# myrrix/myrrix-recommender

Hardware: AMD Instinct MI355X
Metric: ALS rows solved/sec (full iteration) at k=64 (higher is better)
Workload: dtype f32 storage; per-row Gramian: f16x2-split operands (22 bits), f32 accumulate; Cholesky f32

## Files before the change

myrrix-recommender_amd/csrc/als_kernels.h:

```cpp
#pragma once
#include <hip/hip_runtime.h>
#include <stdint.h>

#include <type_traits>

#include "work_plan.h"

namespace mals {

#ifndef MALS_WAVES
#define MALS_WAVES(T, MODE) ((T) <= 4 ? 4 : ((T) == 5 ? 3 : 2))
#endif
#ifndef MALS_WAVES_H
#define MALS_WAVES_H(T, MODE) ((T) <= 2 ? 5 : ((T) <= 4 ? 3 : 2))
#endif

typedef float f32x4 __attribute__((ext_vector_type(4)));
typedef double f64x4 __attribute__((ext_vector_type(4)));

__host__ __device__ constexpr int tri(int T) { return T * (T + 1) / 2; }
__host__ __device__ constexpr int tidx(int T, int i, int j) { return i * T - (i * (i - 1)) / 2 + (j - i); }

constexpr int GRAMIAN_FLUSH_BINADES = 5;
constexpr int YMAX_SLOTS = 64;
// ... 853 lines not shown
    } else {
#pragma unroll
      for (int r = 0; r < 4; ++r) acc[t][r] *= s2;
    }
  }
#pragma unroll
  for (int v = 0; v < T; ++v) bcol[v] *= s2;
  return inv_s2;
}

template <int T, bool PERM = false>
__device__ __forceinline__ void store_row(const SolveParams& p, float (&xcol)[T], float minpiv, float wmax, int row, int lane) {
  if (!(minpiv > p.sing_threshold)) {
    if (lane == 0) {
      if (p.refine_flag) {
        p.refine_flag[row] = 2;
        *p.any_marked = 1;
      } else {
        atomicMin(p.bad_row, (unsigned long long)row);
      }
    }
#pragma unroll
    for (int v = 0; v < T; ++v) xcol[v] = 0.f;
  } else {
    if (minpiv <= 1024.f * p.sing_threshold && lane == 0) {
      const unsigned long long key = ((unsigned long long)__float_as_uint(minpiv) << 32) | (unsigned)row;
      if (key < __builtin_nontemporal_load(p.suspect)) atomicMin(p.suspect, key);
    }
    if (p.refine_flag && p.refine_limit > 0.f && wmax > p.refine_limit * minpiv && lane == 0) {
      p.refine_flag[row] = 1;
      *p.any_marked = 1;
    }
  }
  if constexpr (PERM) {
    static_assert(T == 8, "the permuted feature order belongs to the k = 128 kernels");
    float* o = p.out + (int64_t)row * p.k;
    int l2 = lane;
    asm volatile("" : "+v"(l2));
    const int g = l2 >> 4, c = l2 & 15;
    const bool hi = ((g ^ (c >> 3)) & 1) != 0;
    f32x4 x;
#pragma unroll
    for (int q = 0; q < 4; ++q) x[q] = hi ? xcol[4 + q] : xcol[q];
    if (g < 2) *reinterpret_cast<f32x4*>(o + 8 * c + 4 * g) = x;
  } else {
    float* o = p.out + (int64_t)row * p.k;
    int l2 = lane;
    asm volatile("" : "+v"(l2));
    const int g = l2 >> 4, c = l2 & 15;
#pragma unroll
    for (int m = 0; 4 * m < T; ++m) {
      const float x = select4(g, xcol[4 * m], 4 * m + 1 < T ? xcol[4 * m + 1] : 0.f, 4 * m + 2 < T ? xcol[4 * m + 2] : 0.f,
                              4 * m + 3 < T ? xcol[4 * m + 3] : 0.f);
      const int feat = 16 * (4 * m + g) + c;
      if (4 * m + 3 < T - 1 || feat < p.k) o[feat] = x;
    }
  }
}

template <int T, bool PERM = false>
__device__ __forceinline__ void finish_row(const SolveParams& p, f32x4 (&acc)[tri(T)], const float (&bcol)[T],
                                           int n_u, int row, int lane, float rmax = 0.f) {
  add_ridge<T, PERM>(p, acc, n_u, lane);
  float minpiv = 3.0e38f;
  float xcol[T];
  const float wmax = fmaxf(rmax, p.gramian_weight * __int_as_float(max_entry_bits<T>(acc, lane)));
  cholesky_tiles<T>(acc, lane, minpiv);
  solve_tiles<T>(acc, bcol, xcol, lane);
// ... 1098 lines not shown
```

myrrix-recommender_amd/csrc/lds_kernels.h:

```cpp
#pragma once
#include "als_kernels.h"

namespace mals {

constexpr int LDSK_T = 8, LDSK_E = 8;
#ifndef MALS_LDSK_RESPLIT
#define MALS_LDSK_RESPLIT 1
#endif
constexpr bool LDSK_RESPLIT = MALS_LDSK_RESPLIT != 0;
constexpr int LDSK_ROW_BYTES = 512;
constexpr int LDSK_RING_BYTES = 32 * LDSK_ROW_BYTES;
constexpr int LDSK_CHUNK_BYTES = 512;
constexpr int LDSK_NCHUNK = 3;
constexpr int LDSK_WAVE_BYTES = LDSK_RING_BYTES + LDSK_NCHUNK * LDSK_CHUNK_BYTES;

__host__ __device__ constexpr int ldsk_feature(int v, int c) { return 8 * c + (v ^ (4 * (c >> 3))); }

typedef __attribute__((address_space(3))) char lds_char;

__device__ __forceinline__ void glds16(const void* a, unsigned dst) {
  unsigned keep;
  asm volatile(
      "s_mov_b32 %0, m0\n\t"
      "s_mov_b32 m0, %2\n\ts_nop 0\n\tglobal_load_lds_dwordx4 %1, off\n\t"
      "s_mov_b32 m0, %0"
      : "=&s"(keep)
      : "v"(a), "s"(dst)
      : "memory");
}
__device__ __forceinline__ void glds4x2(const void* a0, const void* a1, unsigned dst) {
  unsigned keep;
  const unsigned d1 = dst + 256;
  asm volatile(
      "s_mov_b32 %0, m0\n\t"
      "s_mov_b32 m0, %3\n\ts_nop 0\n\tglobal_load_lds_dword %1, off nt\n\t"
      "s_mov_b32 m0, %4\n\ts_nop 0\n\tglobal_load_lds_dword %2, off nt\n\t"
      "s_mov_b32 m0, %0"
      : "=&s"(keep)
      : "v"(a0), "v"(a1), "s"(dst), "s"(d1)
      : "memory");
}
template <int N>
__device__ __forceinline__ void wait_vm() {
  asm volatile("s_waitcnt vmcnt(%0)" ::"n"(N) : "memory");
}

typedef const __attribute__((address_space(3))) f32x4* lds_f4;
typedef const __attribute__((address_space(3))) i32x4* lds_i4;
typedef const __attribute__((address_space(3))) float* lds_f1;

struct LdskLane {
  unsigned rd0;
  const char* gsrc;
};

__device__ __forceinline__ void ldsk_chunk_dma(const SolveParams& p, int64_t begin, int len, int base, unsigned buf, int lane) {
  const int n = base + lane;
  const int nn = n < len ? n : len - 1;
  glds4x2(p.col + begin + nn, p.val + begin + nn, buf);
}

__device__ __forceinline__ void ldsk_weights(const SolveParams& p, const lds_char* lds, unsigned buf, int base, int len, int lane, float zscale,
                                             float& w, float& cb) {
  const int widx = 4 * (lane & 15) + (lane >> 4);
  Chunk e;
  e.col = 0;
  e.w = *reinterpret_cast<lds_f1>(lds + buf + 256 + 4 * widx);
  e.cb = base + widx < len ? 1.f : 0.f;
  chunk_weights_h(p, e, zscale);
  w = e.w;
  cb = e.cb;
}

template <int E2>
__device__ __forceinline__ void ldsk_issue_pair(const lds_char* lds, unsigned ring, unsigned cols_at, const LdskLane& L) {
  const i32x4 cols = *reinterpret_cast<lds_i4>(lds + cols_at + 32 * E2);
#pragma unroll
  for (int i = 0; i < 4; ++i) {
    const char* a;
    asm("v_mad_u64_u32 %0, vcc, %1, %2, %3" : "=v"(a) : "v"(cols[i]), "s"((unsigned)LDSK_ROW_BYTES), "v"(L.gsrc) : "vcc");
    glds16(a, ring + 4096 * E2 + 1024 * i);
  }
}
__device__ __forceinline__ unsigned ldsk_cols_addr(unsigned buf_cols, int lane) { return buf_cols + 16 * (unsigned)(lane >> 5); }

template <int E2, int V0>
__device__ __forceinline__ void ldsk_convert_half(const f32x4& ya, const f32x4& yb, float s0, float s1, float c0, float c1,
                                                  ZOp<LDSK_E> (&zh)[LDSK_T], ZOp<LDSK_E> (&zl)[LDSK_T], float (&bpart)[LDSK_T]) {
#pragma unroll
  for (int q = 0; q < 4; ++q) {
    const int v = V0 + q;
    const float y0 = ya[q], y1 = yb[q];
    const float z0 = y0 * s0, z1 = y1 * s1;
    const int hp = pk_rn16(z0, z1);
    const f16x2 hh = __builtin_bit_cast(f16x2, hp);
    zh[v].r[E2] = hp;
    zl[v].r[E2] = pk_rn16(fmaf((float)hh[0], -1.f, z0), fmaf((float)hh[1], -1.f, z1));
    bpart[v] = fmaf(c0, y0, bpart[v]);
    bpart[v] = fmaf(c1, y1, bpart[v]);
  }
}

template <int E2>
__device__ __forceinline__ void ldsk_pair(const lds_char* lds, unsigned ring, float w, float cb, unsigned next_cols, const LdskLane& L,
                                          ZOp<LDSK_E> (&zh)[LDSK_T], ZOp<LDSK_E> (&zl)[LDSK_T], float (&bpart)[LDSK_T]) {
  wait_vm<12>();
  const float s0 = row_bcast<2 * E2>(w), s1 = row_bcast<2 * E2 + 1>(w);
  const float c0 = row_bcast<2 * E2>(cb), c1 = row_bcast<2 * E2 + 1>(cb);
  {
    const f32x4 ya = *reinterpret_cast<lds_f4>(lds + L.rd0 + 4096 * E2);
    const f32x4 yb = *reinterpret_cast<lds_f4>(lds + L.rd0 + 4096 * E2 + 512);
    ldsk_convert_half<E2, 0>(ya, yb, s0, s1, c0, c1, zh, zl, bpart);
  }
  __builtin_amdgcn_sched_barrier(0);
  {
    const f32x4 ya = *reinterpret_cast<lds_f4>(lds + (L.rd0 ^ 16u) + 4096 * E2);
    const f32x4 yb = *reinterpret_cast<lds_f4>(lds + (L.rd0 ^ 16u) + 4096 * E2 + 512);
    ldsk_convert_half<E2, 4>(ya, yb, s0, s1, c0, c1, zh, zl, bpart);
  }
  __builtin_amdgcn_sched_barrier(0);
  ldsk_issue_pair<E2>(lds, ring, next_cols, L);
  __builtin_amdgcn_sched_barrier(0);
}
__device__ __forceinline__ void ldsk_super_step(const lds_char* lds, unsigned ring, float w, float cb, unsigned next_cols, const LdskLane& L,
                                                f32x4 (&acc)[tri(LDSK_T)], float (&bpart)[LDSK_T]) {
  ZOp<LDSK_E> zh[LDSK_T], zl[LDSK_T];
  ldsk_pair<0>(lds, ring, w, cb, next_cols, L, zh, zl, bpart);
  ldsk_pair<1>(lds, ring, w, cb, next_cols, L, zh, zl, bpart);
  ldsk_pair<2>(lds, ring, w, cb, next_cols, L, zh, zl, bpart);
  ldsk_pair<3>(lds, ring, w, cb, next_cols, L, zh, zl, bpart);
  gram_super_step<LDSK_T, LDSK_E>(zh, zl, acc);
  __builtin_amdgcn_sched_barrier(0);
}

__global__ void gramian_perm_kernel(const double* __restrict__ G, int k, float* __restrict__ Gp) {
  constexpr int T = LDSK_T;
  const int e = blockIdx.x * blockDim.x + threadIdx.x;
  if (e >= tri(T) * 256) return;
  const int t = e >> 8, lane = (e >> 2) & 63, reg = e & 3;
  int i = 0, rem = t;
  while (rem >= T - i) {
    rem -= T - i;
    ++i;
  }
  const int j = i + rem;
  const int row = ldsk_feature(i, 4 * (lane >> 4) + reg), col = ldsk_feature(j, lane & 15);
  Gp[e] = (row < k && col < k) ? (float)G[(int64_t)row * k + col] : 0.f;
}

template <int MODE>
__global__ __launch_bounds__(64, 2) void als_lds_kernel_h(SolveParams p) {
  constexpr int T = LDSK_T;
  __shared__ __attribute__((aligned(1024))) char lds_raw[LDSK_WAVE_BYTES];
  const lds_char* lds = (const lds_char*)lds_raw;
  const unsigned lbase = (unsigned)(uintptr_t)lds;
  const int lane = threadIdx.x;
  const int64_t wave = blockIdx.x, n_waves = gridDim.x;
  int64_t it = wave;
  if (it >= p.n_work) return;
  if (p.zscale[2] == 0.f) return;
  const float zscale = __int_as_float(uniform(__float_as_int(p.zscale[0])));
  const float inv_s2 = __int_as_float(uniform(__float_as_int(p.zscale[1])));
  LdskLane L;
  {
    const int g = lane >> 4, c = lane & 15;
    L.rd0 = (unsigned)(g * 1024 + 32 * c + 16 * (c >> 3));
    L.gsrc = reinterpret_cast<const char*>(p.M) + 16 * (lane & 31);
  }
  const unsigned ring = lbase;
  unsigned b_cur = LDSK_RING_BYTES, b_next = LDSK_RING_BYTES + LDSK_CHUNK_BYTES, b_nrow = LDSK_RING_BYTES + 2 * LDSK_CHUNK_BYTES;
  const f32x4* Gp4 = reinterpret_cast<const f32x4*>(p.Gperm);
  WorkItem cur = load_item(p, it);
  WorkItem nxt = load_item(p, it + n_waves);
  WorkItem nx2 = load_item(p, it + 2 * n_waves);
  if (cur.len > 0) {
    ldsk_chunk_dma(p, cur.begin, cur.len, 0, lbase + b_cur, lane);
    if (nxt.len > 0) ldsk_chunk_dma(p, nxt.begin, nxt.len, 0, lbase + b_nrow, lane);
    wait_vm<0>();
    {
      const unsigned ca = ldsk_cols_addr(b_cur, lane);
      ldsk_issue_pair<0>(lds, ring, ca, L);
      ldsk_issue_pair<1>(lds, ring, ca, L);
      ldsk_issue_pair<2>(lds, ring, ca, L);
      ldsk_issue_pair<3>(lds, ring, ca, L);
    }
    for (;;) {
      const WorkItem nx3 = load_item(p, it + 3 * n_waves);
      f32x4 acc[tri(T)];
#pragma unroll
      for (int t = 0; t < tri(T); ++t) acc[t] = f32x4{0.f, 0.f, 0.f, 0.f};
      float bpart[T];
#pragma unroll
      for (int v = 0; v < T; ++v) bpart[v] = 0.f;
#ifdef MALS_PROFILING
      const int64_t trow = it / n_waves - p.trace_start;
      const bool tr = MODE == 0 && p.trace && wave < 64 && trow >= 0 && trow < 64;
      unsigned long long t0 = 0, t1 = 0, t2 = 0;
      if (tr) t0 = __builtin_readcyclecounter();
#endif
      wait_vm<0>();
      const int n_ss = (cur.len + 31) >> 5;
      float w = 0.f, cb = 0.f;
      for (int ss = 0; ss < n_ss; ++ss) {
        const bool odd = ss & 1, last = ss + 1 == n_ss;
        if (!odd) {
          if (ss > 0) {
            const unsigned t = b_cur;
            b_cur = b_next;
            b_next = t;
          }
          ldsk_weights(p, lds, b_cur, 32 * ss, cur.len, lane, zscale, w, cb);
          if (32 * ss + 64 < cur.len) ldsk_chunk_dma(p, cur.begin, cur.len, 32 * ss + 64, lbase + b_next, lane);
        } else {
          w = row_ror<8>(w);
          cb = row_ror<8>(cb);
        }
        const unsigned src = last ? (nxt.len > 0 ? b_nrow : b_cur) : (odd ? b_next : b_cur + 128);
        ldsk_super_step(lds, ring, w, cb, ldsk_cols_addr(src, lane), L, acc, bpart);
      }
#ifdef MALS_PROFILING
      if (tr) t1 = __builtin_readcyclecounter();
#endif
      float bcol[T];
#pragma unroll
      for (int v = 0; v < T; ++v) bcol[v] = reduce_groups(bpart[v], lane);
      {
        const unsigned t = b_cur;
        b_cur = b_nrow;
        b_nrow = t;
      }
      if (nx2.len > 0) ldsk_chunk_dma(p, nx2.begin, nx2.len, 0, lbase + b_nrow, lane);
      if (MODE == 0) {
        const float rmax = p.refine_flag ? __int_as_float(max_entry_bits<T>(acc, lane)) * inv_s2 : 0.f;
        {
          int l2 = lane;
          asm volatile("" : "+v"(l2));
#pragma unroll
          for (int t0 = 0; t0 < tri(T); t0 += 9) {
            f32x4 g4[9];
#pragma unroll
            for (int t = 0; t < 9; ++t) g4[t] = Gp4[(t0 + t) * 64 + l2];
#pragma unroll
            for (int t = 0; t < 9; ++t)
#pragma unroll
              for (int r = 0; r < 4; ++r) acc[t0 + t][r] = fmaf(acc[t0 + t][r], inv_s2, g4[t][r]);
            __builtin_amdgcn_sched_barrier(0);
          }
        }
        add_ridge<T, true>(p, acc, cur.len, lane);
        float minpiv = 3.0e38f, wmax;
        float xcol[T];
        const float inv_s2row = row_scale<T>(acc, bcol, lane, wmax);
        cholesky_tiles<T, true, LDSK_RESPLIT, true>(acc, lane, minpiv);
        minpiv *= inv_s2row;
#ifdef MALS_PROFILING
        if (tr) t2 = __builtin_readcyclecounter();
#endif
        solve_tiles<T>(acc, bcol, xcol, lane);
        store_row<T, true>(p, xcol, minpiv, fmaxf(rmax, p.gramian_weight * wmax), cur.id, lane);
#ifdef MALS_PROFILING
        if (tr) {
          const unsigned long long t3 = __builtin_readcyclecounter();
          if (lane == 0) {
            unsigned long long* o = p.trace + (trow * 64 + wave) * 6;
            o[0] = t0; o[1] = t1; o[2] = t2; o[3] = t3; o[4] = (unsigned long long)cur.len; o[5] = wall_clock64();
          }
        }
#endif
      } else {
        float* s = p.scratch + (int64_t)cur.id * ((tri(T) * 4 + T) * 64);
#pragma unroll
        for (int t = 0; t < tri(T); ++t) reinterpret_cast<f32x4*>(s)[t * 64 + lane] = acc[t] * inv_s2;
#pragma unroll
        for (int v = 0; v < T; ++v) s[(tri(T) * 4 + v) * 64 + lane] = bcol[v];
      }
      cur = nxt;
      nxt = nx2;
      nx2 = nx3;
      it += n_waves;
      if (cur.len <= 0) break;
    }
    wait_vm<0>();
  }
  if (MODE == 0) {
    while (cur.len == 0) {
      f32x4 acc[tri(T)];
#pragma unroll
      for (int t = 0; t < tri(T); ++t) acc[t] = Gp4[t * 64 + lane];
      float bcol[T];
#pragma unroll
      for (int v = 0; v < T; ++v) bcol[v] = 0.f;
      finish_row<T, true>(p, acc, bcol, 0, cur.id, lane);
      it += n_waves;
      cur = load_item(p, it);
    }
  }
}

}
```

myrrix-recommender_amd/csrc/mals_api.hip:

```cpp
#include "../../include/myrrix_als.h"
#include "als_kernels.h"
#include "dual_kernels.h"
#include "lds_kernels.h"
#include "host_eigen.h"
#include "host_solver.h"
#include "mals_internal.h"
#include "mals_handle.h"
#include "hip_buffer.h"
#include "work_plan.h"
#include "convergence.h"

#include <hip/hip_runtime.h>

#include <algorithm>
#include <chrono>
#include <cmath>
#include <cstdio>
#include <cstdlib>
#include <cstring>
#include <limits>
#include <new>
#include <string>
#include <type_traits>
#include <vector>
// ... 270 lines not shown
    double* pd = reinterpret_cast<double*>(s.partials.get() + 2 * slab_bytes);
    int* has2 = reinterpret_cast<int*>(s.partials.get() + 2 * slab_bytes + sizeof(double) * (size_t)GROUPS * tri(T) * 256);
    hipLaunchKernelGGL((gramian_split_kernel<T, false>), dim3((unsigned)(n_slabs / 4)), dim3(256), 0, h->stream, M, n_rows, k,
                       slab_rows, pf, has2, ymax);
    hipLaunchKernelGGL((gramian_split_kernel<T, true>), dim3((unsigned)(n_slabs / 4)), dim3(256), 0, h->stream, M, n_rows, k,
                       slab_rows, pf2, has2, ymax);
    hipLaunchKernelGGL(gramian_reduce_slabs_kernel, dim3((unsigned)((elems + 255) / 256), GROUPS), dim3(256), 0, h->stream, pf, pf2, has2, n_slabs,
                       elems, GROUPS, pd);
    hipLaunchKernelGGL((gramian_finalize_kernel<T, false>), dim3(elems / 64), dim3(256), 0, h->stream, pd, (int64_t)GROUPS, k, G_out, Gf_out);
    HIPCHK(h, hipGetLastError());
    return MALS_OK;
  }
  int64_t n_waves = std::min<int64_t>(1024, std::max<int64_t>(1, (n_rows + 63) / 64));
  n_waves = (n_waves + 3) & ~(int64_t)3;
  int64_t rows_per_wave = (n_rows + n_waves - 1) / n_waves;
  rows_per_wave = std::max<int64_t>(4, (rows_per_wave + 3) & ~(int64_t)3);
  const size_t bytes = sizeof(double) * (size_t)n_waves * tri(T) * 256;
  if (s.partials.capacity() < bytes) HIPCHK(h, s.partials.alloc(bytes));
  double* partials = reinterpret_cast<double*>(s.partials.get());
  if (ymax) HIPCHK(h, hipMemsetAsync(ymax, 0x7f, sizeof(unsigned), h->stream));
  hipLaunchKernelGGL((gramian_partial_kernel<T>), dim3((unsigned)(n_waves / 4)), dim3(256), 0, h->stream, M, n_rows, k,
                     rows_per_wave, partials);
  hipLaunchKernelGGL((gramian_finalize_kernel<T, true, 16>), dim3(elems / 16), dim3(256), 0, h->stream, partials, n_waves,
                     k, G_out, Gf_out);
  HIPCHK(h, hipGetLastError());
  return MALS_OK;
}

int launch_gramian(mals_handle h, SideState& s, const float* M, int64_t n_rows, double* G_out, float* Gf_out, unsigned* ymax = nullptr) {
  return dispatch_T(h, [&](auto t) { return launch_gramian_T<t()>(h, s, M, n_rows, G_out, Gf_out, ymax); });
}

template <typename K>
int persistent_grid(mals_handle h, K kernel, int64_t n_work, unsigned* grid, bool front = false, int block = 256, int resident_per_cu = 0) {
  const int64_t groups = (n_work + block / 64 - 1) / (block / 64);
  if (front) {
    *grid = (unsigned)std::max<int64_t>(1, groups);
    return MALS_OK;
  }
  int per_cu = resident_per_cu;
  if (!per_cu) HIPCHK(h, hipOccupancyMaxActiveBlocksPerMultiprocessor(&per_cu, kernel, 256, 0));
  if (per_cu < 1) per_cu = 1;
  per_cu *= 16;
  if (const char* e = std::getenv("MALS_BLOCKS_PER_CU")) per_cu = std::max(1, std::atoi(e)) * (256 / block);
  const int64_t cap = (int64_t)h->n_cu * per_cu;
  *grid = (unsigned)std::max<int64_t>(1, std::min<int64_t>(groups, cap));
  return MALS_OK;
}

enum { LISTS_ROWS = 1, LISTS_DUAL_ROWS = 2, LISTS_LONG = 4 };

template <typename KR, typename KS, typename KRF, typename KSF, typename KC, typename KCF, typename KP>
struct ListKernels {
  KR rows;
  KS segments;
  KRF rows_f32;
  KSF segments_f32;
  KC finish;
  KCF finish_f32;
  KP prereduce;
  int block;
  int resident_per_cu;
};
template <typename KR, typename KS, typename KRF, typename KSF, typename KC, typename KCF, typename KP>
ListKernels(KR, KS, KRF, KSF, KC, KCF, KP, int, int) -> ListKernels<KR, KS, KRF, KSF, KC, KCF, KP>;

template <typename K, typename KF>
int launch_persistent(mals_handle h, K kernel, KF fallback, int block, int resident_per_cu, const SolveParams& p, int kind, double bytes, bool front) {
  PendingEvent pe;
  unsigned grid = 1;
  if (int rc = persistent_grid(h, kernel, p.n_work, &grid, front, block, resident_per_cu)) return rc;
  if (int rc = begin_timed(h, kind, bytes, pe)) return rc;
  hipLaunchKernelGGL(kernel, dim3(grid), dim3(block), 0, h->stream, p);
  if constexpr (!std::is_same<KF, std::nullptr_t>::value) {
    SolveParams pf = p;
    pf.flags |= 8;
    if (int rc = persistent_grid(h, fallback, p.n_work, &grid)) return rc;
    grid = std::min<unsigned>(grid, (unsigned)h->n_cu * 8u);
    hipLaunchKernelGGL(fallback, dim3(grid), dim3(256), 0, h->stream, pf);
  }
  return end_timed(h, pe);
}

template <typename LK>
int launch_lists(mals_handle h, SideState& s, SolveParams p, int chunk, int which, const LK& fam) {
  const double per = 4.0 * p.k + 8.0;
  const ChunkRange& cr = s.chunks[(size_t)chunk];
  const bool own = which & LISTS_ROWS, longs = which & LISTS_LONG, dual_rows_too = which & LISTS_DUAL_ROWS;
  const WorkItem *A = s.itemsA.get() + cr.offA, *B = s.itemsB.get() + cr.offB;
  const int64_t n_plain = cr.nB - cr.nBand, n_dual = cr.n_dual();
  struct Run {
    const WorkItem* items;
    int64_t n;
    double bytes;
    int kind;
    bool front;
  };
  const Run runs[4] = {
      {B, longs ? n_plain : 0, (double)(cr.nnzB - cr.nnzBand) * per, 1, false},
      {B + n_plain, longs ? cr.nBand : 0, (double)cr.nnzBand * per, 1, s.band_front},
      {A, own ? cr.nA : 0, (double)cr.nnzA * per + (double)cr.nA * per, 0, false},
      {A + cr.nA, dual_rows_too ? n_dual : 0, (double)cr.nnz_dual() * per + (double)n_dual * per, 0, false}};
  for (const Run& r : runs) {
    if (!r.n) continue;
    p.n_work = r.n;
    p.items = r.items;
    if (int rc = r.kind ? launch_persistent(h, fam.segments, fam.segments_f32, fam.block, fam.resident_per_cu, p, 1, r.bytes, r.front)
                        : launch_persistent(h, fam.rows, fam.rows_f32, fam.block, fam.resident_per_cu, p, 0, r.bytes, r.front))
      return rc;
  }
  if (longs && cr.nC) {
    PendingEvent pe;
    if (int rc = begin_timed(h, 2, (double)cr.nC * per, pe)) return rc;
    if (cr.nP) {
      p.n_work = cr.nP;
      p.rowsC = s.rowsC.get() + cr.offP;
      hipLaunchKernelGGL(fam.prereduce, dim3((unsigned)((cr.nP + 3) / 4)), dim3(256), 0, h->stream, p);
    }
    p.n_work = cr.nC;
    p.rowsC = s.rowsC.get() + cr.offC;
    hipLaunchKernelGGL(fam.finish, dim3((unsigned)((cr.nC + 3) / 4)), dim3(256), 0, h->stream, p);
    if constexpr (!std::is_same<decltype(fam.finish_f32), std::nullptr_t>::value) {
      SolveParams pf = p;
      pf.flags |= 8;
      hipLaunchKernelGGL(fam.finish_f32, dim3((unsigned)((cr.nC + 3) / 4)), dim3(256), 0, h->stream, pf);
    }
    if (int rc = end_timed(h, pe)) return rc;
  }
  if (own && cr.nZ) {
    hipLaunchKernelGGL(zero_rows_kernel, dim3((unsigned)((cr.nZ + 31) / 32)), dim3(256), 0, h->stream,
                       A + cr.nA + n_dual, cr.nZ, p.k, p.out);
  }
  HIPCHK(h, hipGetLastError());
  return MALS_OK;
}

template <int T, bool FULL>
int launch_solve_TF(mals_handle h, SideState& s, const SolveParams& p, int chunk, int which) {
  constexpr int D = gather_depth(T);
  constexpr auto rows_f32 = als_persistent_kernel<T, D, 0, FULL>;
  constexpr auto segments_f32 = als_persistent_kernel<T, D, 1, FULL>;
  if constexpr (T == 8 && FULL) {
    if (h->split_f16 && h->lds_gather && p.Gperm)
      return launch_lists(h, s, p, chunk, which, ListKernels{als_lds_kernel_h<0>, als_lds_kernel_h<1>, rows_f32, segments_f32, als_finish_kernel<T, true>,
                                                             als_finish_kernel<T, false>, als_prereduce_kernel<T>, 64, 8});
  }
  if constexpr (T == 4) {
    if (h->split3)
      return launch_lists(h, s, p, chunk, which, ListKernels{als_persistent_kernel_h<T, 0, FULL, 3>, als_persistent_kernel_h<T, 1, FULL, 3>, rows_f32,
                                                             segments_f32, als_finish_kernel<T>, nullptr, als_prereduce_kernel<T>, 256, 0});
  }
  if (h->split_f16)
    return launch_lists(h, s, p, chunk, which, ListKernels{als_persistent_kernel_h<T, 0, FULL>, als_persistent_kernel_h<T, 1, FULL>, rows_f32,
                                                           segments_f32, als_finish_kernel<T>, nullptr, als_prereduce_kernel<T>, 256, 0});
  return launch_lists(h, s, p, chunk, which,
                      ListKernels{rows_f32, segments_f32, nullptr, nullptr, als_finish_kernel<T>, nullptr, als_prereduce_kernel<T>, 256, 0});
}

int launch_solve(mals_handle h, SideState& s, const SolveParams& p, int chunk, int which) {
  return dispatch_T(h, [&](auto t) {
    return p.k == 16 * t() ? launch_solve_TF<t(), true>(h, s, p, chunk, which) : launch_solve_TF<t(), false>(h, s, p, chunk, which);
  });
}

int launch_refine(mals_handle h, const RefineParams& q) {
  const int64_t rows = q.row_end - q.row_begin;
  const unsigned grid = (unsigned)std::max<int64_t>(1, std::min<int64_t>((rows + 255) / 256, (int64_t)h->n_cu * 8));
  return dispatch_T(h, [&](auto t) -> int {
    hipLaunchKernelGGL((als_refine_kernel<t()>), dim3(grid), dim3(256), 0, h->stream, q);
    HIPCHK(h, hipGetLastError());
    return MALS_OK;
  });
}

int launch_gramian_ref(mals_handle h, const SideState& o) {
  const unsigned grid = (unsigned)std::max<int64_t>(1, std::min<int64_t>((o.n_total + 63) / 64, (int64_t)h->n_cu * 2));
  return dispatch_T(h, [&](auto t) -> int {
    hipLaunchKernelGGL(gramian_ref_latch_kernel, dim3(1), dim3(1), 0, h->stream, h->d_gref_state.get());
// ... 415 lines not shown
    case MALS_SOLVE_DUAL: h->dual_blocks = dual_max_blocks(h->T); break;
    default: delete h; return create_fail(MALS_INVALID_ARG, "mals_create: unknown solve_mode");
  }
  if (h->cfg.flags != 0 || !(cfg->alpha > 0.0)) h->dual_blocks = 0;
  {
    hipDeviceProp_t prop;
    if (hipGetDeviceProperties(&prop, cfg->device) == hipSuccess && prop.multiProcessorCount > 0)
      h->n_cu = prop.multiProcessorCount;
  }
  std::memset(&h->stats, 0, sizeof(h->stats));
  h->stats.struct_size = (int32_t)sizeof(mals_stats);
  hipError_t st = hipSetDevice(cfg->device);
  if (st == hipSuccess) st = h->d_bad.alloc(4);
  if (st == hipSuccess) st = h->h_bad.alloc(4);
  if (st == hipSuccess) st = h->d_zscale.alloc(4);
  if (st == hipSuccess) st = h->d_maxabs.alloc(4);
  if (st == hipSuccess) st = h->d_colrange.alloc(2);
  if (st == hipSuccess) st = h->d_refined.alloc(1);
  if (st == hipSuccess) st = h->d_gref_state.alloc(4);
  if (st == hipSuccess) st = hipMemset(h->d_gref_state.get(), 0, 4 * sizeof(int));
  if (st == hipSuccess) st = hipMemset(h->d_refined.get(), 0, sizeof(unsigned long long));
  if (st == hipSuccess) st = hipMemset(h->d_zscale.get(), 0, 4 * sizeof(float));
  if (st == hipSuccess) st = hipMemset(h->d_bad.get(), 0xff, 4 * sizeof(unsigned long long));
  if (st != hipSuccess) {
    delete h;
    return create_fail(MALS_HIP_ERROR, "mals_create: device " + std::to_string(cfg->device) + ": " + hipGetErrorString(st));
  }
  if (const char* e = std::getenv("MALS_REFINE_LIMIT")) h->refine_limit = std::max(0.f, (float)std::atof(e));
  if (hipEventCreateWithFlags(&h->ev_ready, hipEventDisableTiming) != hipSuccess ||
      hipEventCreateWithFlags(&h->ev_refine, hipEventDisableTiming) != hipSuccess) {
    delete h;
    return create_fail(MALS_HIP_ERROR, "mals_create: hipEventCreate failed");
  }
  h->lds_gather = h->cfg.features == 128;
  if (const char* e = std::getenv("MALS_LDS_GATHER")) h->lds_gather = h->lds_gather && std::atoi(e) != 0;
  if (const char* e = std::getenv("MALS_OVERLAP")) h->overlap = std::atoi(e) != 0;
  if (h->overlap) {
    bool ok = hipEventCreateWithFlags(&h->ev_fork, hipEventDisableTiming) == hipSuccess;
    for (int i = 0; i < 2 && ok; ++i)
      ok = hipStreamCreateWithFlags(&h->aux[i], hipStreamNonBlocking) == hipSuccess &&
           hipEventCreateWithFlags(&h->ev_join[i], hipEventDisableTiming) == hipSuccess;
    if (!ok) h->overlap = false;
  }
#ifdef MALS_PROFILING
  if (std::getenv("MALS_DEBUG_TRACE")) {
    (void)h->d_trace.alloc(64 * 64 * 6);
    (void)hipMemset(h->d_trace.get(), 0, 64 * 64 * 6 * sizeof(unsigned long long));
  }
#endif
  t_create_error.clear();
  malsi_serving_create(h);
  *out = h;
  return MALS_OK;
}

int mals_destroy(mals_handle h) {
  if (!h) return MALS_INVALID_ARG;
  (void)hipSetDevice(h->cfg.device);
  malsi_serving_stop_front(h);
  (void)hipStreamSynchronize(h->stream);
  if (h->d_trace) {
    std::vector<unsigned long long> t(64 * 64 * 6);
    (void)hipMemcpy(t.data(), h->d_trace.get(), t.size() * sizeof(unsigned long long), hipMemcpyDeviceToHost);
    for (int r = 0; r < 64; r += 21)
      for (int w = 0; w < 4; w += 1) {
        const unsigned long long* o = &t[(size_t)(r * 64 + w) * 6];
        std::fprintf(stderr, "[trace] iter %2d wave %2d len %5llu gather %7llu chol %7llu solve+store %7llu gap_to_prev_end %lld\n", r, w, o[4],
// ... 399 lines not shown
static int solve_setup(mals_handle h, int side, int chunk_begin, int chunk_end, bool g_to_host) {
  SideState& s = h->side[side];
  SideState& o = h->side[1 - side];
  const int k = h->cfg.features;
  const HalfStamp now{side, o.G_version};
  bool new_half = h->pad != now || h->pad_epoch != o.F_epoch || h->pad_done.size() != s.chunks.size();
  for (int c = chunk_begin; c < chunk_end && !new_half; ++c) new_half = h->pad_done[(size_t)c] != 0;
  if (new_half) {
    h->pad = now;
    h->pad_epoch = o.F_epoch;
    h->pad_done.assign(s.chunks.size(), 0);
    h->tl[0] = now_us();
    h->tl[1] = h->tl[2] = 0.0;
    HIPCHK(h, hipMemsetAsync(h->d_gref_state.get(), 0, 3 * sizeof(int), h->stream));
  }
  for (int c = chunk_begin; c < chunk_end; ++c) h->pad_done[(size_t)c] = 1;
  if (k % 16 != 0) {
    const int ld = 16 * h->T;
    const size_t need = (size_t)o.n_total * (size_t)ld;
    if (need > h->d_Mp.capacity()) {
      new_half = true;
      HIPCHK(h, h->d_Mp.reserve(need, h->stream));
    }
    if (new_half) {
      PendingEvent pe;
      if (int rc = begin_timed(h, 5, (double)o.n_total * 4.0 * (k + ld), pe)) return rc;
      const int64_t n4 = o.n_total * (ld / 4);
      const unsigned blocks = (unsigned)std::min<int64_t>((n4 + 255) / 256, (int64_t)h->n_cu * 32);
      hipLaunchKernelGGL(pad_rows_kernel, dim3(blocks ? blocks : 1), dim3(256), 0, h->stream, o.F, o.n_total, k, ld, h->d_Mp.get());
      HIPCHK(h, hipGetLastError());
      if (int rc = end_timed(h, pe)) return rc;
    }
  }
  if (h->lds_gather && h->split_f16 && k == 128) {
    if (!h->d_Gperm) HIPCHK(h, h->d_Gperm.alloc((size_t)tri(8) * 256));
    if (h->gperm != now) {
      if (h->cfg.flags & MALS_FLAG_LOSS_IGNORES_UNSPECIFIED) {
        HIPCHK(h, hipMemsetAsync(h->d_Gperm.get(), 0, sizeof(float) * (size_t)tri(8) * 256, h->stream));
      } else {
        hipLaunchKernelGGL(gramian_perm_kernel, dim3((unsigned)tri(8)), dim3(256), 0, h->stream, o.G.get(), k, h->d_Gperm.get());
        HIPCHK(h, hipGetLastError());
      }
      h->gperm = now;
    }
  }
  HIPCHK(h, s.refine.reserve((size_t)s.n_local, h->stream));
  if (h->split_f16 && (h->zs != now || h->zs_bound != s.max_abs_val || h->zs_mean != s.mean_abs_val)) {
    const double base_w = (h->cfg.flags & MALS_FLAG_LOSS_IGNORES_UNSPECIFIED) ? 1.0 : 0.0;
    const double w_max = base_w + ((h->cfg.flags & MALS_FLAG_RECONSTRUCT_R) ? 0.0 : std::fabs(h->cfg.alpha) * (double)s.max_abs_val);
    const double w_mean = base_w + ((h->cfg.flags & MALS_FLAG_RECONSTRUCT_R) ? 0.0 : std::fabs(h->cfg.alpha) * s.mean_abs_val);
    int force = -1;
    if (const char* e = std::getenv("MALS_FORCE_RANGE_FLAG")) force = std::atoi(e) != 0;
    hipLaunchKernelGGL(gather_scale_kernel, dim3(1), dim3(64), 0, h->stream, o.G.get(), k, (float)std::sqrt(w_max), (float)std::sqrt(w_mean),
                       (double)o.n_total, force, (o.ymax_version != 0 && o.ymax_version == o.G_version) ? o.d_ymax.get() : nullptr, h->d_zscale.get());
    HIPCHK(h, hipGetLastError());
    h->zs = now;
    h->zs_bound = s.max_abs_val;
    h->zs_mean = s.mean_abs_val;
  }
  if (g_to_host) {
    if (!h->h_G) HIPCHK(h, h->h_G.alloc((size_t)k * k));
    if (!h->ev_G) HIPCHK(h, hipEventCreateWithFlags(&h->ev_G, hipEventDisableTiming));
    HIPCHK(h, hipMemcpyAsync(h->h_G.get(), o.G.get(), sizeof(double) * (size_t)k * k, hipMemcpyDeviceToHost, h->stream));
    HIPCHK(h, hipEventRecord(h->ev_G, h->stream));
  }
  return MALS_OK;
}

static SolveParams solve_params(mals_handle h, int side) {
  SideState& s = h->side[side];
  SideState& o = h->side[1 - side];
  const int k = h->cfg.features;
  SolveParams p;
  p.row_ptr = s.row_ptr;
  p.col = s.col;
  p.val = s.val;
  p.M = o.F;
  p.ldm = k;
  if (k % 16 != 0) {
    p.M = h->d_Mp.get();
    p.ldm = 16 * h->T;
  }
  p.Gf = o.Gf.get();
  p.Gperm = h->lds_gather && h->split_f16 && k == 128 ? h->d_Gperm.get() : nullptr;
  p.out = s.F + s.row_offset * k;
  p.items = nullptr;
  p.rowsC = s.rowsC.get();
  p.scratch = s.scratch.get();
  p.bad_row = h->d_bad.get() + side;
  p.suspect = h->d_bad.get() + 2 + side;
  p.any_marked = h->d_gref_state.get();
  p.refine_flag = s.refine.get();
  p.refine_limit = (h->cfg.flags & MALS_FLAG_LOSS_IGNORES_UNSPECIFIED) ? h->refine_limit / 16.f : h->refine_limit;
  p.gramian_weight = 0.25f;
  if (h->cfg.flags & MALS_FLAG_RECONSTRUCT_R) {
    p.gramian_weight = 1.f;
    p.refine_limit *= 0.25f;
  }
  p.n_work = 0;
  p.trace = h->d_trace.get();
  p.trace_start = 0;
  if (const char* ts = std::getenv("MALS_DEBUG_TRACE")) p.trace_start = std::atoi(ts);
  if (const char* ts = std::getenv("MALS_DEBUG_TRACE_SIDE")) if (std::atoi(ts) != side) p.trace = nullptr;
  p.k = k;
  p.flags = h->cfg.flags;
  p.alpha = (float)h->cfg.alpha;
  p.lambda_alpha = (float)(h->cfg.lambda * h->cfg.alpha);
  p.sing_threshold = (float)h->cfg.singularity_threshold;
  p.zscale = h->d_zscale.get();
  return p;
}

static int solve_one_chunk(mals_handle h, int side, const SolveParams& p, int c, int phase, bool want_dual, bool prepare_dual, bool* dual_now) {
  SideState& s = h->side[side];
  const SideState& o = h->side[1 - side];
  const ChunkRange& cr = s.chunks[(size_t)c];
  const bool resume = phase == SOLVE_END;
// ... 507 lines not shown
```

Baseline: 139.4 million.

## Extend LDS-gather DMA row kernel to k=64 with templated tile count

Templates the LDS ring-buffer gather kernel on the tile count T, so the k=64 case (T=4) also uses global_load_lds DMA of neighbour factor rows into an LDS ring, with a permuted Gramian image and its own write-back path. The k=64 row work now dispatches to this new kernel while segments stay on the register kernel, run with a separate block size. The goal is to overlap factor-row gathers with the f16-split Gramian math, as the k=128 path already does. It adds an optional dynamic LDS pad knob for tuning occupancy, and in exchange brings new code paths and different occupancy behaviour at k=64.

```diff
diff --git a/myrrix-recommender_amd/csrc/als_kernels.h b/myrrix-recommender_amd/csrc/als_kernels.h
--- a/myrrix-recommender_amd/csrc/als_kernels.h
+++ b/myrrix-recommender_amd/csrc/als_kernels.h
@@ -909,8 +909,13 @@
       *p.any_marked = 1;
     }
   }
-  if constexpr (PERM) {
-    static_assert(T == 8, "the permuted feature order belongs to the k = 128 kernels");
+  if constexpr (PERM && T == 4) {
+    float* o = p.out + (int64_t)row * p.k;
+    int l2 = lane;
+    asm volatile("" : "+v"(l2));
+    if (l2 < 16) *reinterpret_cast<f32x4*>(o + 4 * l2) = f32x4{xcol[0], xcol[1], xcol[2], xcol[3]};
+  } else if constexpr (PERM) {
+    static_assert(T == 8, "the permuted feature orders belong to the k = 64 and k = 128 kernels");
     float* o = p.out + (int64_t)row * p.k;
     int l2 = lane;
     asm volatile("" : "+v"(l2));
diff --git a/myrrix-recommender_amd/csrc/lds_kernels.h b/myrrix-recommender_amd/csrc/lds_kernels.h
--- a/myrrix-recommender_amd/csrc/lds_kernels.h
+++ b/myrrix-recommender_amd/csrc/lds_kernels.h
@@ -3,18 +3,25 @@
 
 namespace mals {
 
-constexpr int LDSK_T = 8, LDSK_E = 8;
+constexpr int LDSK_E = 8;
 #ifndef MALS_LDSK_RESPLIT
 #define MALS_LDSK_RESPLIT 1
 #endif
 constexpr bool LDSK_RESPLIT = MALS_LDSK_RESPLIT != 0;
-constexpr int LDSK_ROW_BYTES = 512;
-constexpr int LDSK_RING_BYTES = 32 * LDSK_ROW_BYTES;
 constexpr int LDSK_CHUNK_BYTES = 512;
 constexpr int LDSK_NCHUNK = 3;
-constexpr int LDSK_WAVE_BYTES = LDSK_RING_BYTES + LDSK_NCHUNK * LDSK_CHUNK_BYTES;
-
-__host__ __device__ constexpr int ldsk_feature(int v, int c) { return 8 * c + (v ^ (4 * (c >> 3))); }
+__host__ __device__ constexpr int ldsk_row_bytes(int T) { return 64 * T; }
+__host__ __device__ constexpr int ldsk_ring_bytes(int T) { return 32 * ldsk_row_bytes(T); }
+__host__ __device__ constexpr int ldsk_pair_bytes(int T) { return 8 * ldsk_row_bytes(T); }
+__host__ __device__ constexpr int ldsk_wave_bytes(int T) { return ldsk_ring_bytes(T) + LDSK_NCHUNK * LDSK_CHUNK_BYTES; }
+__host__ __device__ constexpr int ldsk_pair_loads(int T) { return ldsk_pair_bytes(T) / 1024; }
+__host__ __device__ constexpr int ldsk_waves_per_simd(int T) { return T == 8 ? 2 : 4; }
+
+template <int T>
+__host__ __device__ constexpr int ldsk_feature(int v, int c) {
+  static_assert(T == 8 || T == 4, "feature orders exist for k = 128 and k = 64");
+  return T == 8 ? 8 * c + (v ^ (4 * (c >> 3))) : 4 * c + v;
+}
 
 typedef __attribute__((address_space(3))) char lds_char;
 
@@ -47,12 +54,26 @@
 
 typedef const __attribute__((address_space(3))) f32x4* lds_f4;
 typedef const __attribute__((address_space(3))) i32x4* lds_i4;
+typedef const __attribute__((address_space(3))) int* lds_i1;
 typedef const __attribute__((address_space(3))) float* lds_f1;
 
 struct LdskLane {
   unsigned rd0;
   const char* gsrc;
 };
+template <int T>
+__device__ __forceinline__ LdskLane ldsk_lane(const SolveParams& p, int lane) {
+  LdskLane L;
+  if constexpr (T == 8) {
+    const int g = lane >> 4, c = lane & 15;
+    L.rd0 = (unsigned)(g * 1024 + 32 * c + 16 * (c >> 3));
+    L.gsrc = reinterpret_cast<const char*>(p.M) + 16 * (lane & 31);
+  } else {
+    L.rd0 = 16u * (unsigned)lane;
+    L.gsrc = reinterpret_cast<const char*>(p.M) + 16 * (lane & 15);
+  }
+  return L;
+}
 
 __device__ __forceinline__ void ldsk_chunk_dma(const SolveParams& p, int64_t begin, int len, int base, unsigned buf, int lane) {
   const int n = base + lane;
@@ -72,21 +93,33 @@
   cb = e.cb;
 }
 
-template <int E2>
+template <int T, int E2>
 __device__ __forceinline__ void ldsk_issue_pair(const lds_char* lds, unsigned ring, unsigned cols_at, const LdskLane& L) {
-  const i32x4 cols = *reinterpret_cast<lds_i4>(lds + cols_at + 32 * E2);
-#pragma unroll
-  for (int i = 0; i < 4; ++i) {
+  constexpr int N = ldsk_pair_loads(T);
+  int cols[N];
+  if constexpr (T == 8) {
+    const i32x4 c4 = *reinterpret_cast<lds_i4>(lds + cols_at + 32 * E2);
+#pragma unroll
+    for (int i = 0; i < 4; ++i) cols[i] = c4[i];
+  } else {
+#pragma unroll
+    for (int i = 0; i < 2; ++i) cols[i] = *reinterpret_cast<lds_i1>(lds + cols_at + 32 * E2 + 16 * i);
+  }
+#pragma unroll
+  for (int i = 0; i < N; ++i) {
     const char* a;
-    asm("v_mad_u64_u32 %0, vcc, %1, %2, %3" : "=v"(a) : "v"(cols[i]), "s"((unsigned)LDSK_ROW_BYTES), "v"(L.gsrc) : "vcc");
-    glds16(a, ring + 4096 * E2 + 1024 * i);
-  }
-}
-__device__ __forceinline__ unsigned ldsk_cols_addr(unsigned buf_cols, int lane) { return buf_cols + 16 * (unsigned)(lane >> 5); }
-
-template <int E2, int V0>
+    asm("v_mad_u64_u32 %0, vcc, %1, %2, %3" : "=v"(a) : "v"(cols[i]), "s"((unsigned)ldsk_row_bytes(T)), "v"(L.gsrc) : "vcc");
+    glds16(a, ring + ldsk_pair_bytes(T) * E2 + 1024 * i);
+  }
+}
+template <int T>
+__device__ __forceinline__ unsigned ldsk_cols_addr(unsigned buf_cols, int lane) {
+  return T == 8 ? buf_cols + 16 * (unsigned)(lane >> 5) : buf_cols + 4 * (unsigned)(lane >> 4);
+}
+
+template <int T, int E2, int V0>
 __device__ __forceinline__ void ldsk_convert_half(const f32x4& ya, const f32x4& yb, float s0, float s1, float c0, float c1,
-                                                  ZOp<LDSK_E> (&zh)[LDSK_T], ZOp<LDSK_E> (&zl)[LDSK_T], float (&bpart)[LDSK_T]) {
+                                                  ZOp<LDSK_E> (&zh)[T], ZOp<LDSK_E> (&zl)[T], float (&bpart)[T]) {
 #pragma unroll
   for (int q = 0; q < 4; ++q) {
     const int v = V0 + q;
@@ -101,40 +134,48 @@
   }
 }
 
-template <int E2>
+template <int T, int E2>
 __device__ __forceinline__ void ldsk_pair(const lds_char* lds, unsigned ring, float w, float cb, unsigned next_cols, const LdskLane& L,
-                                          ZOp<LDSK_E> (&zh)[LDSK_T], ZOp<LDSK_E> (&zl)[LDSK_T], float (&bpart)[LDSK_T]) {
-  wait_vm<12>();
+                                          ZOp<LDSK_E> (&zh)[T], ZOp<LDSK_E> (&zl)[T], float (&bpart)[T]) {
+  constexpr int PB = ldsk_pair_bytes(T);
+  wait_vm<3 * ldsk_pair_loads(T)>();
   const float s0 = row_bcast<2 * E2>(w), s1 = row_bcast<2 * E2 + 1>(w);
   const float c0 = row_bcast<2 * E2>(cb), c1 = row_bcast<2 * E2 + 1>(cb);
-  {
-    const f32x4 ya = *reinterpret_cast<lds_f4>(lds + L.rd0 + 4096 * E2);
-    const f32x4 yb = *reinterpret_cast<lds_f4>(lds + L.rd0 + 4096 * E2 + 512);
-    ldsk_convert_half<E2, 0>(ya, yb, s0, s1, c0, c1, zh, zl, bpart);
+  if constexpr (T == 8) {
+    {
+      const f32x4 ya = *reinterpret_cast<lds_f4>(lds + L.rd0 + PB * E2);
+      const f32x4 yb = *reinterpret_cast<lds_f4>(lds + L.rd0 + PB * E2 + 512);
+      ldsk_convert_half<T, E2, 0>(ya, yb, s0, s1, c0, c1, zh, zl, bpart);
+    }
+    __builtin_amdgcn_sched_barrier(0);
+    {
+      const f32x4 ya = *reinterpret_cast<lds_f4>(lds + (L.rd0 ^ 16u) + PB * E2);
+      const f32x4 yb = *reinterpret_cast<lds_f4>(lds + (L.rd0 ^ 16u) + PB * E2 + 512);
+      ldsk_convert_half<T, E2, 4>(ya, yb, s0, s1, c0, c1, zh, zl, bpart);
+    }
+  } else {
+    const f32x4 ya = *reinterpret_cast<lds_f4>(lds + L.rd0 + PB * E2);
+    const f32x4 yb = *reinterpret_cast<lds_f4>(lds + L.rd0 + PB * E2 + 1024);
+    ldsk_convert_half<T, E2, 0>(ya, yb, s0, s1, c0, c1, zh, zl, bpart);
   }
   __builtin_amdgcn_sched_barrier(0);
-  {
-    const f32x4 ya = *reinterpret_cast<lds_f4>(lds + (L.rd0 ^ 16u) + 4096 * E2);
-    const f32x4 yb = *reinterpret_cast<lds_f4>(lds + (L.rd0 ^ 16u) + 4096 * E2 + 512);
-    ldsk_convert_half<E2, 4>(ya, yb, s0, s1, c0, c1, zh, zl, bpart);
-  }
+  ldsk_issue_pair<T, E2>(lds, ring, next_cols, L);
   __builtin_amdgcn_sched_barrier(0);
-  ldsk_issue_pair<E2>(lds, ring, next_cols, L);
+}
+template <int T>
+__device__ __forceinline__ void ldsk_super_step(const lds_char* lds, unsigned ring, float w, float cb, unsigned next_cols, const LdskLane& L,
+                                                f32x4 (&acc)[tri(T)], float (&bpart)[T]) {
+  ZOp<LDSK_E> zh[T], zl[T];
+  ldsk_pair<T, 0>(lds, ring, w, cb, next_cols, L, zh, zl, bpart);
+  ldsk_pair<T, 1>(lds, ring, w, cb, next_cols, L, zh, zl, bpart);
+  ldsk_pair<T, 2>(lds, ring, w, cb, next_cols, L, zh, zl, bpart);
+  ldsk_pair<T, 3>(lds, ring, w, cb, next_cols, L, zh, zl, bpart);
+  gram_super_step<T, LDSK_E>(zh, zl, acc);
   __builtin_amdgcn_sched_barrier(0);
 }
-__device__ __forceinline__ void ldsk_super_step(const lds_char* lds, unsigned ring, float w, float cb, unsigned next_cols, const LdskLane& L,
-                                                f32x4 (&acc)[tri(LDSK_T)], float (&bpart)[LDSK_T]) {
-  ZOp<LDSK_E> zh[LDSK_T], zl[LDSK_T];
-  ldsk_pair<0>(lds, ring, w, cb, next_cols, L, zh, zl, bpart);
-  ldsk_pair<1>(lds, ring, w, cb, next_cols, L, zh, zl, bpart);
-  ldsk_pair<2>(lds, ring, w, cb, next_cols, L, zh, zl, bpart);
-  ldsk_pair<3>(lds, ring, w, cb, next_cols, L, zh, zl, bpart);
-  gram_super_step<LDSK_T, LDSK_E>(zh, zl, acc);
-  __builtin_amdgcn_sched_barrier(0);
-}
-
-__global__ void gramian_perm_kernel(const double* __restrict__ G, int k, float* __restrict__ Gp) {
-  constexpr int T = LDSK_T;
+
+template <int T>
+__device__ __forceinline__ void gramian_perm_image(const double* __restrict__ G, int k, float* __restrict__ Gp) {
   const int e = blockIdx.x * blockDim.x + threadIdx.x;
   if (e >= tri(T) * 256) return;
   const int t = e >> 8, lane = (e >> 2) & 63, reg = e & 3;
@@ -144,14 +185,19 @@
     ++i;
   }
   const int j = i + rem;
-  const int row = ldsk_feature(i, 4 * (lane >> 4) + reg), col = ldsk_feature(j, lane & 15);
+  const int row = ldsk_feature<T>(i, 4 * (lane >> 4) + reg), col = ldsk_feature<T>(j, lane & 15);
   Gp[e] = (row < k && col < k) ? (float)G[(int64_t)row * k + col] : 0.f;
 }
-
-template <int MODE>
-__global__ __launch_bounds__(64, 2) void als_lds_kernel_h(SolveParams p) {
-  constexpr int T = LDSK_T;
-  __shared__ __attribute__((aligned(1024))) char lds_raw[LDSK_WAVE_BYTES];
+__global__ void gramian_perm_kernel(const double* __restrict__ G, int k, float* __restrict__ Gp) { gramian_perm_image<8>(G, k, Gp); }
+__global__ void gramian_perm64_kernel(const double* __restrict__ G, int k, float* __restrict__ Gp) { gramian_perm_image<4>(G, k, Gp); }
+
+template <int T, int MODE>
+__device__ __forceinline__ void ldsk_rows(const SolveParams& p) {
+  static_assert(T == 8 || MODE == 0, "k = 64: the segments stay with the register kernel (partial slots in plain feature order)");
+  constexpr int RING = ldsk_ring_bytes(T);
+  constexpr int GPASS = T == 8 ? 9 : 5;
+  static_assert(tri(T) % GPASS == 0, "whole passes");
+  __shared__ __attribute__((aligned(1024))) char lds_raw[ldsk_wave_bytes(T)];
   const lds_char* lds = (const lds_char*)lds_raw;
   const unsigned lbase = (unsigned)(uintptr_t)lds;
   const int lane = threadIdx.x;
@@ -161,14 +207,9 @@
   if (p.zscale[2] == 0.f) return;
   const float zscale = __int_as_float(uniform(__float_as_int(p.zscale[0])));
   const float inv_s2 = __int_as_float(uniform(__float_as_int(p.zscale[1])));
-  LdskLane L;
-  {
-    const int g = lane >> 4, c = lane & 15;
-    L.rd0 = (unsigned)(g * 1024 + 32 * c + 16 * (c >> 3));
-    L.gsrc = reinterpret_cast<const char*>(p.M) + 16 * (lane & 31);
-  }
+  const LdskLane L = ldsk_lane<T>(p, lane);
   const unsigned ring = lbase;
-  unsigned b_cur = LDSK_RING_BYTES, b_next = LDSK_RING_BYTES + LDSK_CHUNK_BYTES, b_nrow = LDSK_RING_BYTES + 2 * LDSK_CHUNK_BYTES;
+  unsigned b_cur = RING, b_next = RING + LDSK_CHUNK_BYTES, b_nrow = RING + 2 * LDSK_CHUNK_BYTES;
   const f32x4* Gp4 = reinterpret_cast<const f32x4*>(p.Gperm);
   WorkItem cur = load_item(p, it);
   WorkItem nxt = load_item(p, it + n_waves);
@@ -178,11 +219,11 @@
     if (nxt.len > 0) ldsk_chunk_dma(p, nxt.begin, nxt.len, 0, lbase + b_nrow, lane);
     wait_vm<0>();
     {
-      const unsigned ca = ldsk_cols_addr(b_cur, lane);
-      ldsk_issue_pair<0>(lds, ring, ca, L);
-      ldsk_issue_pair<1>(lds, ring, ca, L);
-      ldsk_issue_pair<2>(lds, ring, ca, L);
-      ldsk_issue_pair<3>(lds, ring, ca, L);
+      const unsigned ca = ldsk_cols_addr<T>(b_cur, lane);
+      ldsk_issue_pair<T, 0>(lds, ring, ca, L);
+      ldsk_issue_pair<T, 1>(lds, ring, ca, L);
+      ldsk_issue_pair<T, 2>(lds, ring, ca, L);
+      ldsk_issue_pair<T, 3>(lds, ring, ca, L);
     }
     for (;;) {
       const WorkItem nx3 = load_item(p, it + 3 * n_waves);
@@ -216,7 +257,7 @@
           cb = row_ror<8>(cb);
         }
         const unsigned src = last ? (nxt.len > 0 ? b_nrow : b_cur) : (odd ? b_next : b_cur + 128);
-        ldsk_super_step(lds, ring, w, cb, ldsk_cols_addr(src, lane), L, acc, bpart);
+        ldsk_super_step<T>(lds, ring, w, cb, ldsk_cols_addr<T>(src, lane), L, acc, bpart);
       }
 #ifdef MALS_PROFILING
       if (tr) t1 = __builtin_readcyclecounter();
@@ -236,12 +277,12 @@
           int l2 = lane;
           asm volatile("" : "+v"(l2));
 #pragma unroll
-          for (int t0 = 0; t0 < tri(T); t0 += 9) {
-            f32x4 g4[9];
-#pragma unroll
-            for (int t = 0; t < 9; ++t) g4[t] = Gp4[(t0 + t) * 64 + l2];
-#pragma unroll
-            for (int t = 0; t < 9; ++t)
+          for (int t0 = 0; t0 < tri(T); t0 += GPASS) {
+            f32x4 g4[GPASS];
+#pragma unroll
+            for (int t = 0; t < GPASS; ++t) g4[t] = Gp4[(t0 + t) * 64 + l2];
+#pragma unroll
+            for (int t = 0; t < GPASS; ++t)
 #pragma unroll
               for (int r = 0; r < 4; ++r) acc[t0 + t][r] = fmaf(acc[t0 + t][r], inv_s2, g4[t][r]);
             __builtin_amdgcn_sched_barrier(0);
@@ -251,7 +292,8 @@
         float minpiv = 3.0e38f, wmax;
         float xcol[T];
         const float inv_s2row = row_scale<T>(acc, bcol, lane, wmax);
-        cholesky_tiles<T, true, LDSK_RESPLIT, true>(acc, lane, minpiv);
+        if constexpr (T == 8) cholesky_tiles<T, true, LDSK_RESPLIT, true>(acc, lane, minpiv);
+        else cholesky_tiles<T, true>(acc, lane, minpiv);
         minpiv *= inv_s2row;
 #ifdef MALS_PROFILING
         if (tr) t2 = __builtin_readcyclecounter();
@@ -297,4 +339,12 @@
   }
 }
 
-}
+template <int MODE>
+__global__ __launch_bounds__(64, ldsk_waves_per_simd(8)) void als_lds_kernel_h(SolveParams p) {
+  ldsk_rows<8, MODE>(p);
+}
+__global__ __launch_bounds__(64, ldsk_waves_per_simd(4)) void als_lds64_kernel_h(SolveParams p) {
+  ldsk_rows<4, 0>(p);
+}
+
+}
diff --git a/myrrix-recommender_amd/csrc/mals_api.hip b/myrrix-recommender_amd/csrc/mals_api.hip
--- a/myrrix-recommender_amd/csrc/mals_api.hip
+++ b/myrrix-recommender_amd/csrc/mals_api.hip
@@ -326,14 +326,15 @@
 }
 
 template <typename K>
-int persistent_grid(mals_handle h, K kernel, int64_t n_work, unsigned* grid, bool front = false, int block = 256, int resident_per_cu = 0) {
+int persistent_grid(mals_handle h, K kernel, int64_t n_work, unsigned* grid, bool front = false, int block = 256, int resident_per_cu = 0,
+                    size_t lds_pad = 0) {
   const int64_t groups = (n_work + block / 64 - 1) / (block / 64);
   if (front) {
     *grid = (unsigned)std::max<int64_t>(1, groups);
     return MALS_OK;
   }
   int per_cu = resident_per_cu;
-  if (!per_cu) HIPCHK(h, hipOccupancyMaxActiveBlocksPerMultiprocessor(&per_cu, kernel, 256, 0));
+  if (!per_cu) HIPCHK(h, hipOccupancyMaxActiveBlocksPerMultiprocessor(&per_cu, kernel, 256, lds_pad));
   if (per_cu < 1) per_cu = 1;
   per_cu *= 16;
   if (const char* e = std::getenv("MALS_BLOCKS_PER_CU")) per_cu = std::max(1, std::atoi(e)) * (256 / block);
@@ -355,6 +356,7 @@
   KP prereduce;
   int block;
   int resident_per_cu;
+  int segments_block = 0, segments_resident_per_cu = 0;
 };
 template <typename KR, typename KS, typename KRF, typename KSF, typename KC, typename KCF, typename KP>
 ListKernels(KR, KS, KRF, KSF, KC, KCF, KP, int, int) -> ListKernels<KR, KS, KRF, KSF, KC, KCF, KP>;
@@ -363,9 +365,12 @@
 int launch_persistent(mals_handle h, K kernel, KF fallback, int block, int resident_per_cu, const SolveParams& p, int kind, double bytes, bool front) {
   PendingEvent pe;
   unsigned grid = 1;
-  if (int rc = persistent_grid(h, kernel, p.n_work, &grid, front, block, resident_per_cu)) return rc;
+  size_t lds_pad = 0;
+  if (kind == 0)
+    if (const char* e = std::getenv("MALS_ROWS_LDS_PAD")) lds_pad = (size_t)std::max(0, std::atoi(e));
+  if (int rc = persistent_grid(h, kernel, p.n_work, &grid, front, block, resident_per_cu, lds_pad)) return rc;
   if (int rc = begin_timed(h, kind, bytes, pe)) return rc;
-  hipLaunchKernelGGL(kernel, dim3(grid), dim3(block), 0, h->stream, p);
+  hipLaunchKernelGGL(kernel, dim3(grid), dim3(block), lds_pad, h->stream, p);
   if constexpr (!std::is_same<KF, std::nullptr_t>::value) {
     SolveParams pf = p;
     pf.flags |= 8;
@@ -399,7 +404,8 @@
     if (!r.n) continue;
     p.n_work = r.n;
     p.items = r.items;
-    if (int rc = r.kind ? launch_persistent(h, fam.segments, fam.segments_f32, fam.block, fam.resident_per_cu, p, 1, r.bytes, r.front)
+    if (int rc = r.kind ? launch_persistent(h, fam.segments, fam.segments_f32, fam.segments_block ? fam.segments_block : fam.block,
+                                            fam.segments_block ? fam.segments_resident_per_cu : fam.resident_per_cu, p, 1, r.bytes, r.front)
                         : launch_persistent(h, fam.rows, fam.rows_f32, fam.block, fam.resident_per_cu, p, 0, r.bytes, r.front))
       return rc;
   }
@@ -438,6 +444,14 @@
     if (h->split_f16 && h->lds_gather && p.Gperm)
       return launch_lists(h, s, p, chunk, which, ListKernels{als_lds_kernel_h<0>, als_lds_kernel_h<1>, rows_f32, segments_f32, als_finish_kernel<T, true>,
                                                              als_finish_kernel<T, false>, als_prereduce_kernel<T>, 64, 8});
+  }
+  if constexpr (T == 4 && FULL) {
+    if (h->split_f16 && !h->split3 && h->lds_gather && p.Gperm) {
+      ListKernels fam{als_lds64_kernel_h, als_persistent_kernel_h<T, 1, FULL>, rows_f32, segments_f32, als_finish_kernel<T>, nullptr,
+                      als_prereduce_kernel<T>, 64, 4 * ldsk_waves_per_simd(4)};
+      fam.segments_block = 256;
+      return launch_lists(h, s, p, chunk, which, fam);
+    }
   }
   if constexpr (T == 4) {
     if (h->split3)
@@ -919,7 +933,7 @@
     delete h;
     return create_fail(MALS_HIP_ERROR, "mals_create: hipEventCreate failed");
   }
-  h->lds_gather = h->cfg.features == 128;
+  h->lds_gather = h->cfg.features == 128 || h->cfg.features == 64;
   if (const char* e = std::getenv("MALS_LDS_GATHER")) h->lds_gather = h->lds_gather && std::atoi(e) != 0;
   if (const char* e = std::getenv("MALS_OVERLAP")) h->overlap = std::atoi(e) != 0;
   if (h->overlap) {
@@ -1385,13 +1399,14 @@
       if (int rc = end_timed(h, pe)) return rc;
     }
   }
-  if (h->lds_gather && h->split_f16 && k == 128) {
+  if (h->lds_gather && h->split_f16 && (k == 128 || (k == 64 && !h->split3))) {
     if (!h->d_Gperm) HIPCHK(h, h->d_Gperm.alloc((size_t)tri(8) * 256));
     if (h->gperm != now) {
       if (h->cfg.flags & MALS_FLAG_LOSS_IGNORES_UNSPECIFIED) {
         HIPCHK(h, hipMemsetAsync(h->d_Gperm.get(), 0, sizeof(float) * (size_t)tri(8) * 256, h->stream));
       } else {
-        hipLaunchKernelGGL(gramian_perm_kernel, dim3((unsigned)tri(8)), dim3(256), 0, h->stream, o.G.get(), k, h->d_Gperm.get());
+        if (k == 128) hipLaunchKernelGGL(gramian_perm_kernel, dim3((unsigned)tri(8)), dim3(256), 0, h->stream, o.G.get(), k, h->d_Gperm.get());
+        else hipLaunchKernelGGL(gramian_perm64_kernel, dim3((unsigned)tri(4)), dim3(256), 0, h->stream, o.G.get(), k, h->d_Gperm.get());
         HIPCHK(h, hipGetLastError());
       }
       h->gperm = now;
@@ -1435,7 +1450,7 @@
     p.ldm = 16 * h->T;
   }
   p.Gf = o.Gf.get();
-  p.Gperm = h->lds_gather && h->split_f16 && k == 128 ? h->d_Gperm.get() : nullptr;
+  p.Gperm = h->lds_gather && h->split_f16 && (k == 128 || (k == 64 && !h->split3)) ? h->d_Gperm.get() : nullptr;
   p.out = s.F + s.row_offset * k;
   p.items = nullptr;
   p.rowsC = s.rowsC.get();
```

New measurement: 140.9 million, median of 6. 1.01x the previous value.
